# daac-tools/daachorse

Measured on AMD Instinct MI355X. Metric: haystack GB/s scanned (find_overlapping_iter(..).count(), 100k-pattern bytewise automaton), higher is better.
Workload: dtype u8/u32 integer

## Files before the change

### daachorse_amd/csrc/api_internal.hpp

```cpp
#pragma once
#include <hip/hip_runtime.h>

#include <algorithm>
#include <atomic>
#include <cassert>
#include <cstdlib>
#include <chrono>
#include <cstring>
#include <map>
#include <memory>
#include <condition_variable>
#include <deque>
#include <functional>
#include <mutex>
#include <string>
#include <thread>
#include <utility>
#include <vector>

#include "charwise.hpp"
#include "device_tables.hpp"
#include "gram.hpp"
#include "gram2.hpp"
#include "gram4.hpp"
// ... 12 lines not shown
    X(rows_share_pct, 45, 1)                                                                                                                 \
    X(blocks_per_cu, 0, 0)                                                                                                     \
    X(threads, 1024, 0)                                                                                                                      \
    X(iter_window, 64ll << 20, 0)                  \
    X(max_result_bytes, 8ll << 30, 0)                                                                                                        \
    X(gram_lds_budget, 158 * 1024, 1)                                                                                                        \
    X(gram_region, 0, 0)                                          \
    X(gram_slab, 4096, 0)                                                                                                                    \
    X(gram_ppl, 0, 0)                                                                      \
    X(gram_dense, -1, 0)                                                                                      \
    X(gram_rank_in_lds, -1, 1)                                                                                \
    X(gram_version, 0, 0)                   \
    X(gram4_arith, 1, 0)                  \
    X(gram4_filter, 1, 0)                      \
    X(gram4_mph, 8, 1)                    \
    X(gram2_dpp, 1, 0)                                                  \
    X(find3, 1, 0)                                                                                         \
    X(pfx_probe, 16384, 0)                                                             \
    X(pfx, 1, 1)                                 \
    X(gram_tail, -1, 0)                         \
    X(gram2_rfull, 1, 0)                                                            \
    X(emit, 1, 0)                            \
    X(emit_rec_per_kib, 32, 0)                               \
    X(restart_bpc, 8, 0)                                                              \
    X(restart_chain, 1, 0)                      \
    X(chain_rounds, 24, 0)                                                                                                                   \
    X(overlap_micro, 1, 0)                \
    X(pool, 1, 0)                                                                 \
    X(pool_keep, 0, 0)                                                                    \
    X(left3, 1, 0)                        \
// ... 397 lines not shown
```

### daachorse_amd/csrc/api_scan.hip

```cpp
#include "api_internal.hpp"

static daac_status scan_count_impl(daac_pma *pma, int mode, int engine, const uint8_t *hay, size_t len, size_t begin, int hay_is_device,
                                   void *stream_, uint64_t *count, uint64_t *checksum, uint64_t *result_dev, bool want_checksum);

namespace {

__global__ void repack8_kernel(const uint4 *in, uint2 *out, unsigned long long n, unsigned long long base, uint32_t end_bits) {
    for (unsigned long long i = static_cast<unsigned long long>(blockIdx.x) * blockDim.x + threadIdx.x; i < n; i += static_cast<unsigned long long>(gridDim.x) * blockDim.x) {
        const uint4 t = in[i];
        const unsigned long long end = (static_cast<unsigned long long>(t.y) << 32) | t.x;
        out[i] = uint2{t.w, static_cast<uint32_t>(end - base) | (t.z << end_bits)};
    }
}
__global__ void repack16_kernel(const daac_match *in, uint4 *out, unsigned long long n) {
    for (unsigned long long i = static_cast<unsigned long long>(blockIdx.x) * blockDim.x + threadIdx.x; i < n; i += static_cast<unsigned long long>(gridDim.x) * blockDim.x) {
        const daac_match m = in[i];
        out[i] = uint4{static_cast<uint32_t>(m.end), static_cast<uint32_t>(m.end >> 32), static_cast<uint32_t>(m.end - m.start), m.value};
    }
}

__global__ void shard_subtract_kernel(unsigned long long *r, const unsigned long long *h, unsigned long long from32) {
    r[0] -= h[0];
    r[1] -= h[1];
    r[2] -= h[2];
// ... 307 lines not shown
    return DAAC_OK;
}

daac_status stage_window(const uint8_t *host_hay, uint64_t copy_from, uint64_t end, hipStream_t stream, void **dbuf,
                         const uint8_t **virt_base) {
    const uint64_t n = end - copy_from;
    const uint64_t skew = copy_from & 15;
    HIP_TRY(hipMalloc(dbuf, n + skew + 32));
    if (n) HIP_TRY(hipMemcpyAsync(static_cast<uint8_t *>(*dbuf) + skew, host_hay + copy_from, n, hipMemcpyHostToDevice, stream));
    *virt_base = static_cast<const uint8_t *>(*dbuf) + skew - copy_from;
    return DAAC_OK;
}


static bool gram4_shape(const DeviceTables *t, CountPlan &cp) {
    const bool want_rfull = OPT(gram2_rfull) != 0, want_arith = OPT(gram4_arith) != 0, want_filter = OPT(gram4_filter) != 0;
    const uint32_t waves = static_cast<uint32_t>(OPT(threads)) > 512 ? 16u : 8u;
    const int64_t ppl_opt = OPT(gram_ppl);
    struct Shape { uint32_t ppl; bool rfull; } shapes[4] = {{32u, true}, {32u, false}, {16u, true}, {16u, false}};
    for (uint32_t w = waves; w >= 8u; w >>= 1)
        for (const Shape &sh : shapes)
            if ((sh.ppl == ppl_opt || (ppl_opt != 16 && ppl_opt != 32)) && (want_rfull || !sh.rfull) &&
                gram4_plan(t->gram4, sh.ppl, w, sh.rfull, want_arith, want_filter, 160u * 1024u, cp.g4)) { cp.ppl = sh.ppl; return true; }
    return false;
}

CountPlan resolve_count(const daac_pma *pma, const DeviceTables *t, int mode, int engine, bool want_checksum, uint64_t span) {
    CountPlan cp{};
    auto refuse = [&](const char *err, CountKernel kernel = CountKernel::walkers) { cp.kernel = kernel; cp.st = DAAC_ERR_UNSUPPORTED; cp.err = err; return cp; };
    const int64_t gv = OPT(gram_version);
    const bool g1_can = t->gram_ok && gv != 2;
    const bool g2_can = t->gram2_ok && (!want_checksum || t->gram2.exact_ok) && gv != 1 && !(gv == 0 && want_checksum && g1_can);
    const bool gw_can = t->gramw_ok && (!want_checksum || t->gramw.exact_ok);
    const bool applies = !pma->charwise && mode == DAAC_FIND_OVERLAPPING && pma->host.is_standard() && span < (1ull << 35);
    const bool gram = applies && (engine == DAAC_ENGINE_GRAM || (engine == DAAC_ENGINE_AUTO && (g2_can || g1_can || gw_can)));
    bool pfx = applies && t->pfx_ok && (engine == DAAC_ENGINE_PFX || (engine == DAAC_ENGINE_AUTO && !gram));
    cp.probe = pfx && engine == DAAC_ENGINE_AUTO && OPT(pfx_probe) != 0;
    if (cp.probe && t->pfx_dense.load() > 0) pfx = false;
// ... 28 lines not shown
std::pair<int, int> count_ids(const DeviceTables *t, const CountPlan &cp) {
    switch (cp.kernel) {
    case CountKernel::gram4: return {DAAC_ENGINE_GRAM, DAAC_KERNEL_GRAM_COUNT};
    case CountKernel::gram: case CountKernel::gram2: return {DAAC_ENGINE_GRAM, DAAC_KERNEL_GRAM_EXACT};
    case CountKernel::gram2w: return {DAAC_ENGINE_GRAM, DAAC_KERNEL_GRAM_WIDE};
    case CountKernel::pfx: return {DAAC_ENGINE_PFX, DAAC_KERNEL_PFX};
    default: return {cp.tier ? DAAC_ENGINE_TIERED : DAAC_ENGINE_DARRAY, micro_walker(t, cp.charwise, cp.tier) ? DAAC_KERNEL_MICRO : DAAC_KERNEL_SEGMENT};
    }
}

static std::string count_kernel_name(const CountPlan &cp) {
    static const char *const family[] = {"gram4", "gram", "gram2", "gram2w", "pfx"};
    if (cp.kernel == CountKernel::walkers) return cp.charwise ? "charwise" : cp.tier ? "tiered" : "darray";
    if (cp.kernel != CountKernel::gram4) return family[static_cast<int>(cp.kernel)];
    return "gram4 ppl=" + std::to_string(cp.ppl) + " dir=" + std::to_string(cp.g4.dir) + " waves=" + std::to_string(cp.g4.threads / 64) + " arith=" +
           std::to_string(cp.g4.arith) + " filter=" + std::to_string(cp.g4.filter) + " mph=" + std::to_string(cp.g4.mph) + " tail=" + (OPT(gram_tail) < 0 ? std::string("auto") : std::to_string(OPT(gram_tail) > 0 ? 1 : 0));
}

}
}

extern "C" {

static daac_status scan_count_impl(daac_pma *pma, int mode, int engine, const uint8_t *hay, size_t len, size_t begin, int hay_is_device,
                                   void *stream_, uint64_t *count, uint64_t *checksum, uint64_t *result_dev, bool want_checksum) {
    PmaScope scope_(pma);
    if (!pma || (len && !hay) || (!result_dev && (!count || (want_checksum && !checksum))) || begin > len) {
        set_error("bad argument");
        return DAAC_ERR_INVALID_ARGUMENT;
    }
    hipStream_t stream = static_cast<hipStream_t>(stream_);
// ... 409 lines not shown
```

### daachorse_amd/csrc/api_upload.hip

```cpp
#include "api_internal.hpp"

namespace {

bool recover_patterns(const HostPma &p, std::vector<uint8_t> &blob, std::vector<uint64_t> &offs, std::vector<uint32_t> &vals) {
    const uint32_t n = static_cast<uint32_t>(p.states_len());
    if (n == 0 || output_pos_of(p.opos_ch(kRoot)) != 0) return false;
    constexpr uint32_t kNone = 0xffffffffu;
    std::vector<uint32_t> depth(n, kNone), parent(n, kNone), order{kRoot};
    std::vector<uint8_t> label(n, 0);
    depth[kRoot] = 0;
    for (size_t qi = 0; qi < order.size(); ++qi) {
        const uint32_t s = order[qi], base = p.base(s);
        if (base == 0) continue;
        for (uint32_t c = 0; c < 256; ++c) {
            const uint32_t t = base ^ c;
            if (t >= n || t == kRoot || t == kDead || check_of(p.opos_ch(t)) != c) continue;
            if (depth[t] != kNone) return false;
            depth[t] = depth[s] + 1; parent[t] = s; label[t] = static_cast<uint8_t>(c);
            order.push_back(t);
        }
    }
    blob.clear(); offs.assign(1, 0); vals.clear();
    std::vector<uint8_t> tmp;
    for (const uint32_t s : order) {
// ... 314 lines not shown
            d.lds_exact = d.off_ring_exact + ring_bytes;
            if (d.off_m_exact + d.m_bytes > (1u << 17) || d.lds_exact > 160u * 1024u) exact_ok = false;
            d.K = g2.K; d.C = g2.C; d.s16 = g2.s16; d.unused_byte = g2.unused_byte;
            d.n_deep = static_cast<uint32_t>(g2.dhit.size());
            d.exact_ok = exact_ok;
            d.xlane_dpp = OPT(gram2_dpp) != 0;
            t->gram2_ok = d.off_m_count + d.m_bytes <= (1u << 17) && d.lds_count <= 160u * 1024u;
            if (t->gram2_ok) {
                Gram4Tables g4;
                build_gram4_tables(g2, g4);
                Gram4Dev &q = t->gram4;
                q = Gram4Dev{};
                if ((st = t->put(g4.cls, q.cls)) != DAAC_OK) return st;
                if ((st = t->put(g4.m, q.m)) != DAAC_OK) return st;
                q.m_bytes = p16(g4.m.size() * 4);
                if (g4.s16) {
                    std::vector<uint16_t> s16(g4.sdir.begin(), g4.sdir.end());
                    const uint16_t *ps;
                    if ((st = t->put(s16, ps)) != DAAC_OK) return st;
                    q.sdir = ps;
                    q.s_bytes = p16(s16.size() * 2);
                    if ((st = t->put(g4.rfull, q.rfull)) != DAAC_OK) return st;
                    q.rfull_bytes = p16(g4.rfull.size() * 2);
                } else {
                    const uint32_t *ps;
                    if ((st = t->put(g4.sdir, ps)) != DAAC_OK) return st;
                    q.sdir = ps;
                    q.s_bytes = p16(g4.sdir.size() * 4);
                }
                { const U32x2 *x; if ((st = t->put(g4.dhit_c, x)) != DAAC_OK) return st; q.dhit_c = reinterpret_cast<const uint2 *>(x); }
// ... 446 lines not shown
```

### daachorse_amd/csrc/device_tables.hpp

```cpp
#pragma once

#include <hip/hip_runtime.h>

#include <cstdint>

#include "../../include/daachorse_amd.h"
#include "gram4_mph.hpp"

namespace daac {

struct TierDev {
    const void *rows;
    const uint32_t *bcmap;
    const uint32_t *bfail;
    const uint2 *ssum;
    const uint8_t *cls;
    const uint4 *grec;
    const uint32_t *sopos;
    const uint32_t *outputs;
    const uint32_t *ohash;
    uint32_t C, NA, NB, N;
    uint32_t off_bcmap, off_bfail, off_ssum, off_cls, lds_bytes;
    uint32_t row32, root_flag;
};
// ... 146 lines not shown
    uint32_t v3c_bytes, v3c_dir, v3c_val;
};
hipError_t launch_gram2_scan(const Gram2Dev &dev, const GramArgs &a, bool exact, uint32_t blocks, uint32_t threads, hipStream_t stream);

struct Gram3Lds {
    uint32_t off_s;
    uint32_t off_wave;
    uint32_t wave_stride;
    uint32_t lds_bytes, threads, rfull;
};

constexpr uint32_t kGram4EndsBitDev = 30;
struct Gram4Dev {
    const uint8_t *cls;
    const uint32_t *m;
    const uint16_t *rfull;
    const void *sdir;
    const uint2 *dhit_c;
    const uint4 *dhit_t;
    const uint4 *drec_c;
    const uint4 *drec_t;
    const uint32_t *bloom;
    uint32_t bloom_words;
    const uint8_t *mph_disp;
    const uint2 *dhit_h;
    G4Mph mph;
    uint32_t mph_bytes;
    uint32_t m_bytes, rfull_bytes, s_bytes;
    uint32_t K, C, s16, arith, lo, unused_byte, n_deep;
};
struct Gram4Lds {
    uint32_t off_wave;
    uint32_t wave_stride;
    uint32_t off_cls;
    uint32_t off_s;
    uint32_t off_m;
    uint32_t s_bytes;
    uint32_t lds_bytes, threads;
    uint32_t arith;
    uint32_t dir;
    uint32_t filter;
    uint32_t off_b;
    uint32_t s_bytes_f;
    uint32_t mph;
};
uint32_t gram4_filter_room(uint32_t m_bytes, uint32_t sdir_bytes, bool arith, uint32_t lds_limit);
bool gram4_plan(const Gram4Dev &dev, uint32_t ppl, uint32_t waves, bool rfull, bool want_arith, bool want_filter, uint32_t lds_limit, Gram4Lds &L);
hipError_t launch_gram4_scan(const Gram4Dev &dev, const GramArgs &a, const Gram4Lds &L, uint32_t blocks, hipStream_t stream);

constexpr uint32_t kEmit3Tile = 1024;
constexpr uint32_t kEmit3Chunk = 1024;
constexpr uint32_t kEmit3MaxExtrasAtPosition = 15;
constexpr uint32_t kEmit3MaxExtras = 64;
constexpr uint32_t kEmit3Stage = 960;
constexpr uint32_t kEmit3ExpandWave = (kEmit3Stage + 64) * 8 + 2048 + 256 + 1024 + kEmit3MaxExtras * 16 + 16;
constexpr uint32_t kEmit3ExpandWave16 = (kEmit3Stage + 64) * 2 + 1040 + 2048 + 256 + 1024 + kEmit3MaxExtras * 16 + 16;
struct Emit3Args {
    const uint8_t *hay_al;
    uint32_t lead;
    uint32_t vlen;
    uint32_t emit_from;
    uint8_t *ann;
// ... 125 lines not shown
```

### daachorse_amd/csrc/gram4.cpp

```cpp
#include "gram4.hpp"

#include <algorithm>

namespace daac {

void build_gram4_tables(const Gram2Tables &g2, Gram4Tables &out) {
    out = Gram4Tables{};
    if (!g2.available) return;
    const uint32_t K = g2.K, C = g2.C, OTH = C - 1;
    auto perm = [&](uint32_t c) -> uint32_t { return c == 0 ? OTH : c - 1; };
    out.K = K;
    out.C = C;
    out.unused_byte = g2.unused_byte;
    out.cls.resize(256);
    for (uint32_t b = 0; b < 256; ++b) out.cls[b] = static_cast<uint8_t>(perm(g2.cls[b]));
    {
        uint32_t lo = 256;
        for (uint32_t b = 0; b < 256; ++b) if (out.cls[b] == 0) lo = b;
        bool ok = lo < 256;
        for (uint32_t b = 0; b < 256 && ok; ++b) {
            const uint32_t u = b - lo;
            ok = out.cls[b] == (u < OTH ? u : OTH);
        }
        out.arith = ok;
// ... 190 lines not shown
            if (d == 256) ok = false;
            else disp[b] = static_cast<uint8_t>(d);
        }
        if (!ok) continue;
        t.mph = p;
        t.mph_seed = seed;
        t.mph_slots = slots;
        t.mph_disp = disp;
        t.dhit_h.assign(slots, U32x2{0u, 0u});
        for (size_t i = 0; i < n; ++i) t.dhit_h[g4m_slot(h[i], f[i], disp[g4m_bucket(h[i], p)], p)] = t.dhit_c[i];
        return true;
    }
    return false;
}

}
```

### daachorse_amd/csrc/gram4.hpp

```cpp
#pragma once

#include <cstdint>
#include <vector>

#include "gram2.hpp"
#include "gram4_filter.hpp"
#include "gram4_mph.hpp"

namespace daac {

struct Gram4Tables {
    bool available = false;
    uint32_t K = 0, C = 0;
    bool arith = false;
    uint32_t lo = 0;
    uint8_t unused_byte = 0;
    bool s16 = false;
    std::vector<uint8_t> cls;
    std::vector<uint32_t> m;
    std::vector<uint16_t> rfull;
    std::vector<uint32_t> sdir;
    std::vector<U32x2> dhit_c;
    std::vector<U32x4> dhit_t, drec_c, drec_t;
    std::vector<uint32_t> bloom;
    uint32_t filter_keys = 0;
    std::vector<uint8_t> mph_disp;
    std::vector<U32x2> dhit_h;
    uint32_t mph_slots = 0, mph_seed = 0;
    G4Mph mph{};
};

constexpr uint32_t kGram4EndsBit = 30;
constexpr uint32_t kGram4ChildBits = 0x3fffffffu;

void build_gram4_tables(const Gram2Tables &g2, Gram4Tables &out);
bool build_gram4_filter(Gram4Tables &t, uint32_t max_bytes);
constexpr uint32_t kGram4MphSeeds = 8;
bool build_gram4_mph(Gram4Tables &t, uint32_t max_disp_bytes, uint32_t max_seeds = kGram4MphSeeds);

}
```

### daachorse_amd/csrc/gram4_kernels.hip

```cpp
#include <hip/hip_runtime.h>

#include <algorithm>
#include <cstdint>
#include <utility>

#include "device_tables.hpp"
#include "gram4_filter.hpp"

namespace daac {

namespace {

typedef uint32_t g4_u32x4_t __attribute__((ext_vector_type(4)));
constexpr uint32_t kList4 = 256;
constexpr uint32_t kProbePercent4 = 3;
typedef __attribute__((address_space(3))) const uint32_t lds4_cu32;
typedef __attribute__((address_space(3))) uint32_t lds4_u32;
typedef __attribute__((address_space(3))) const uint16_t lds4_cu16;
typedef __attribute__((address_space(3))) uint16_t lds4_u16;
typedef __attribute__((address_space(3))) const uint8_t lds4_cu8;
typedef __attribute__((address_space(3))) g4_u32x4_t lds4_u32x4;

__device__ __forceinline__ uint32_t pin4(uint32_t x) {
    asm("" : "+v"(x));
    return x;
}
__device__ __forceinline__ uint32_t mad24(uint32_t a, uint32_t b, uint32_t c) {
    uint32_t d;
    asm("v_mad_u32_u24 %0, %1, %2, %3" : "=v"(d) : "v"(a), "s"(b), "v"(c));
    return d;
}
__device__ __forceinline__ uint32_t wave_shr1_4(uint32_t v, uint32_t lane0) {
    uint32_t d = lane0;
    asm volatile("s_nop 1\nv_mov_b32_dpp %0, %1 wave_shr:1 row_mask:0xf bank_mask:0xf" : "+v"(d) : "v"(v));
    return d;
}
__device__ __forceinline__ uint32_t g4_wave_scan(uint32_t v) {
    v += static_cast<uint32_t>(__builtin_amdgcn_update_dpp(0, static_cast<int>(v), 0x111, 0xf, 0xf, false));
    v += static_cast<uint32_t>(__builtin_amdgcn_update_dpp(0, static_cast<int>(v), 0x112, 0xf, 0xf, false));
    v += static_cast<uint32_t>(__builtin_amdgcn_update_dpp(0, static_cast<int>(v), 0x114, 0xf, 0xf, false));
    v += static_cast<uint32_t>(__builtin_amdgcn_update_dpp(0, static_cast<int>(v), 0x118, 0xf, 0xf, false));
    v += static_cast<uint32_t>(__builtin_amdgcn_update_dpp(0, static_cast<int>(v), 0x142, 0xa, 0xf, false));
    v += static_cast<uint32_t>(__builtin_amdgcn_update_dpp(0, static_cast<int>(v), 0x143, 0xc, 0xf, false));
    return v;
}
template <typename F, int... I>
__device__ __forceinline__ void g4_turns(F &&f, std::integer_sequence<int, I...>) {
    (void)(... && f(std::integral_constant<int, I>{}));
}
__device__ __forceinline__ unsigned long long g4_wave_sum(unsigned long long v) {
#pragma unroll
    for (int off = 32; off > 0; off >>= 1) v += __shfl_down(v, off, 64);
    return v;
}
__device__ __forceinline__ void g4_copy(void *dst, const void *src, uint32_t bytes) {
    const uint4 *s = reinterpret_cast<const uint4 *>(src);
    uint4 *d = reinterpret_cast<uint4 *>(dst);
    for (uint32_t i = threadIdx.x; i < bytes / 16; i += blockDim.x) d[i] = s[i];
}
__device__ __forceinline__ void g4_reduce(unsigned long long cnt, unsigned long long *scratch, unsigned long long *result) {
    const unsigned long long c = g4_wave_sum(cnt);
    __syncthreads();
    const int wave = threadIdx.x >> 6, lane = threadIdx.x & 63;
    if (lane == 0) scratch[wave] = c;
    __syncthreads();
    if (threadIdx.x == 0) {
        unsigned long long r0 = 0;
        for (int w = 0; w < static_cast<int>((blockDim.x + 63) >> 6); ++w) r0 += scratch[w];
        if (r0) atomicAdd(result, r0);
    }
}

}

template <int K, int Q, bool ARITH, int DIR, bool TAIL, bool FILT, bool MPH = false>
__device__ __forceinline__ void gram4_body(const Gram4Dev &g, const GramArgs &a, const Gram4Lds &L, char *smem) {
    static_assert(!(FILT && TAIL), "the filter runs in front of the plain records");
    static_assert(!(FILT && DIR == 0), "the filter's Bloom array lies where the per-word directory would");
    static_assert(!MPH || FILT, "the perfect hash serves the survivors of the filter");
    constexpr int P = 16 * Q;
    constexpr int GS = 8;
    constexpr uint32_t SB = 64u * P;
    constexpr uint32_t SLOT = SB + 32u;
    const uint32_t offM = L.off_m, offS = L.off_s, offC = L.off_cls;
    const uint32_t lo = g.lo, OTH = g.C - 1u, C = g.C;
    auto cls_of = [&](uint32_t byte) -> uint32_t {
        if (ARITH) {
            const uint32_t u = byte - lo;
            return u < OTH ? u : OTH;
        }
        return *reinterpret_cast<lds4_cu8 *>(static_cast<uintptr_t>(offC + byte));
    };
    auto lds_u32 = [&](uint32_t addr) -> uint32_t { return *reinterpret_cast<lds4_cu32 *>(static_cast<uintptr_t>(addr)); };
    auto below = [&](uint32_t k) -> uint32_t { return (1u << k) - 1u; };

    const uint32_t lane = threadIdx.x & 63;
    const uint32_t lane_off = pin4(lane * (16u * Q));
    const uint32_t wave_in_wg = __builtin_amdgcn_readfirstlane(threadIdx.x >> 6);
    const uint32_t C4 = C * 4u, CC4 = C * C * 4u;
    const uint32_t ub4 = g.unused_byte * 0x01010101u;
    const uint8_t *__restrict__ hay = a.hay_al;
    const uint64_t nwaves = static_cast<uint64_t>(gridDim.x) * (blockDim.x >> 6);
    const uint32_t tb = L.off_wave + wave_in_wg * L.wave_stride;
    const uint32_t listb = wave_in_wg * (kList4 * 2u);
    const uint64_t slab_index = (static_cast<uint64_t>(blockIdx.x) * (blockDim.x >> 6) + wave_in_wg) * a.wq_slab;
    uint4 *__restrict__ slab4 = reinterpret_cast<uint4 *>(a.wq) + slab_index;
    uint32_t wq_n = 0, slab_hi = 0;
    uint64_t epoch_base = 0;
    const uint32_t drain_early = wave_in_wg * 64u;

    unsigned long long tot_cnt = 0;
    uint32_t cnt32 = 0;

    auto load_chunk = [&](uint64_t v) -> uint4 {
// ... 195 lines not shown
        if (ARITH) {
            idx = mad24((x_lo >> 8) & 0xffu, C, ((x_lo >> 16) & 0xffu) - lo_idx);
            if (K == 3) idx = mad24(x_lo & 0xffu, C * C, idx);
            d = (x_lo >> 24) - lo;
        } else {
            const uint32_t c1 = cls_of((x_lo >> 8) & 0xffu), c2 = cls_of((x_lo >> 16) & 0xffu);
            d = cls_of(x_lo >> 24);
            idx = __umul24(c1, C) + c2;
            if (K == 3) idx = __umul24(cls_of(x_lo & 0xffu), C * C) + idx;
        }
        const uint32_t am = (idx << 2) + offM;
        const uint32_t own = lds_u32(am);
        uint32_t rank;
        if (DIR == 0) {
            const uint32_t base = *reinterpret_cast<lds4_cu16 *>(static_cast<uintptr_t>((idx << 1) + offS));
            rank = base + __popc(own & below(d));
        } else {
            const uint32_t grp = am & ~15u;
            const uint32_t qx = lds_u32(grp), qy = lds_u32(grp + 4u), qz = lds_u32(grp + 8u);
            const uint32_t gi = pin4(idx >> 2);
            const uint32_t base = DIR == 1 ? *reinterpret_cast<lds4_cu16 *>(static_cast<uintptr_t>((gi << 1) + offS))
                                           : *reinterpret_cast<lds4_cu32 *>(static_cast<uintptr_t>((gi << 2) + offS));
            const uint32_t mx = static_cast<uint32_t>(__builtin_amdgcn_sbfe(static_cast<int>(0xEEEEEEEEu), idx, 1u));
            const uint32_t my = static_cast<uint32_t>(__builtin_amdgcn_sbfe(static_cast<int>(0xCCCCCCCCu), idx, 1u));
            const uint32_t mz = static_cast<uint32_t>(__builtin_amdgcn_sbfe(static_cast<int>(0x88888888u), idx, 1u));
            uint32_t under = __popc(own & below(d));
            under += __popc(qx & mx & 0x3fffffffu);
            under += __popc(qy & my & 0x3fffffffu);
            under += __popc(qz & mz & 0x3fffffffu);
            rank = base + under;
        }
        if (TAIL) {
            pend = g.dhit_t[rank];
        } else {
            const uint2 h = g.dhit_c[rank];
            pend = uint4{h.x, h.y, 0u, 0u};
        }
    };
    const G4Mph mph = g.mph;
    auto hash_and_ask = [&](uint32_t x_lo) {
        const uint32_t x = K == 3 ? x_lo : x_lo >> 8;
        const uint32_t h = g4f_h(x);
        const uint32_t d = *reinterpret_cast<lds4_cu8 *>(static_cast<uintptr_t>(offS + g4m_bucket(h, mph)));
        const uint2 r = g.dhit_h[g4m_slot(h, g4m_f(x, mph), d, mph)];
// ... 49 lines not shown
            pend_t0 = 0;
            pend_t1 = 0;
        }
        pend_valid = true;
    };

    uint64_t region = static_cast<uint64_t>(blockIdx.x) * (blockDim.x >> 6) + wave_in_wg;
    while (region < a.nregions) {
      slab_hi = static_cast<uint32_t>((region * a.region_bytes) >> 31);
      epoch_base = static_cast<uint64_t>(slab_hi) << 31;
      for (; region < a.nregions && static_cast<uint32_t>((region * a.region_bytes) >> 31) == slab_hi; region += nwaves) {
        const uint64_t rbase = region * a.region_bytes;
        const uint64_t rend = rbase + a.region_bytes < a.vlen ? rbase + a.region_bytes : a.vlen;
        uint32_t carry = 0, tail4 = 0;
#pragma unroll
        for (int i = 0; i < K; ++i) carry |= (rbase >= static_cast<uint64_t>(K - i) ? cls_of(raw_at(rbase - (K - i))) : OTH) << (8 * i);
#pragma unroll
        for (int i = 0; i < 4; ++i) tail4 |= (rbase >= static_cast<uint64_t>(4 - i) ? raw_at(rbase - (4 - i)) : static_cast<uint32_t>(g.unused_byte)) << (8 * i);
        tail4 = __builtin_amdgcn_readfirstlane(tail4);
        carry = __builtin_amdgcn_readfirstlane(carry);
        uint32_t mcarry;
        {
            uint32_t x = (((carry >> (8 * (K - 1))) & 0xffu) << 2) + offM;
            x += __umul24((carry >> (8 * (K - 2))) & 0xffu, C4);
            if (K == 3) x += __umul24(carry & 0xffu, CC4);
            mcarry = __builtin_amdgcn_readfirstlane(lds_u32(x));
        }

        const uint32_t rlen = static_cast<uint32_t>(rend - rbase);
        const uint32_t fast_lo = rbase < 16u ? SB : 0u;
        const uint32_t fast_hi = rlen & ~(SB - 1u);
        auto fetch = [&](uint32_t off, uint4 (&out)[Q]) {
            if (off >= fast_lo && off < fast_hi) {
                const uint8_t *__restrict__ base = hay + rbase + off;
                uint32_t voff = lane_off;
                asm volatile("" : "+v"(voff));
#pragma unroll
                for (int q = 0; q < Q; ++q) {
                    const g4_u32x4_t t = __builtin_nontemporal_load(reinterpret_cast<const g4_u32x4_t *>(base + voff + 16u * q));
                    out[q] = uint4{t.x, t.y, t.z, t.w};
                }
                return;
// ... 34 lines not shown
#pragma unroll
            for (int q = 0; q < Q; ++q)
                *reinterpret_cast<lds4_u32x4 *>(static_cast<uintptr_t>(my_text + 16u * q)) = g4_u32x4_t{cur[q].x, cur[q].y, cur[q].z, cur[q].w};
            if (lane == 0) {
                *reinterpret_cast<lds4_u32 *>(static_cast<uintptr_t>(slot + 12u)) = tail4;
                *reinterpret_cast<lds4_u32x4 *>(static_cast<uintptr_t>(slot + 16u + SB)) = g4_u32x4_t{pf0[0].x, pf0[0].y, pf0[0].z, pf0[0].w};
            }
            tail4 = __builtin_amdgcn_readlane(cur[Q - 1].w, 63);

            uint32_t kx[K + P];
#pragma unroll
            for (int q = 0; q < Q; ++q) {
                const uint32_t w[4] = {cur[q].x, cur[q].y, cur[q].z, cur[q].w};
#pragma unroll
                for (int b = 0; b < 16; ++b) {
                    kx[K + 16 * q + b] = pin4(cls_of((w[b >> 2] >> (8 * (b & 3))) & 0xffu));
                    __builtin_assume(kx[K + 16 * q + b] < 32u);
                }
            }
            uint32_t pk = 0;
#pragma unroll
            for (int i = 0; i < K; ++i) pk |= kx[P + i] << (8 * i);
            const uint32_t left = wave_shr1_4(pk, carry);
            carry = __builtin_amdgcn_readlane(pk, 63);
#pragma unroll
            for (int i = 0; i < K; ++i) { kx[i] = (left >> (8 * i)) & 0xffu; __builtin_assume(kx[i] < 32u); }

            uint32_t H = 0, ccnt = 0, roll = 0, mprev = 0;
#pragma unroll
            for (int grp = 0; grp < P / GS; ++grp) {
                uint32_t mw[GS];
#pragma unroll
                for (int jj = 0; jj < GS; ++jj) {
                    const int j = grp * GS + jj;
                    uint32_t x = pin4((kx[K + j] << 2) + offM);
                    x = mad24(kx[K + j - 1], C4, x);
                    if (K == 3) x = mad24(kx[K + j - 2], CC4, x);
                    mw[jj] = lds_u32(x);
                }
#pragma unroll
                for (int jj = 0; jj < GS; ++jj) {
                    const int j = grp * GS + jj;
                    roll = __builtin_amdgcn_alignbit(roll, mw[jj], 30);
                    if (j > 0) H = __builtin_amdgcn_alignbit((jj == 0 ? mprev : mw[jj - 1]) >> kx[K + j], H, 1);
                    if ((j & 15) == 15) {
                        ccnt += __popc(roll & 0x55555555u) + 2u * __popc(roll & 0xaaaaaaaau);
                        roll = 0;
                    }
                }
                mprev = mw[GS - 1];
            }
            {
                const uint32_t mleft = wave_shr1_4(mprev, mcarry);
                mcarry = __builtin_amdgcn_readlane(mprev, 63);
                H |= __builtin_amdgcn_ubfe(mleft, kx[K], 1) << (32 - P);
            }
            cnt32 += ccnt;

            const uint32_t text_adj = my_text - (32u - P) - tb;
            for (;;) {
                if (__ballot(H != 0u) == 0) break;
                const uint32_t n = __popc(H);
                const uint32_t incl = g4_wave_scan(n);
                const uint32_t tot = __builtin_amdgcn_readlane(incl, 63);
                const uint32_t first = q_tail + incl - n;
                const uint32_t room = first < kList4 ? kList4 - first : 0u;
                const uint32_t lim = n < room ? n : room;
                const uint32_t at = pin4(listb + (first << 1));
                g4_turns([&](auto tc) -> bool {
                    constexpr uint32_t t = decltype(tc)::value;
// ... 20 lines not shown
        }
        tot_cnt += cnt32;
        cnt32 = 0;
      }
      if (st_n + q_tail - q_head != 0) process_batch(st_n + q_tail - q_head);
      if (FILT && sb_n != 0) { survivors_ask(sb_n); sb_n = 0; }
      consume_pending();
      finish_second();
      drain();
      tot_cnt += cnt32;
      cnt32 = 0;
    }
    g4_reduce(tot_cnt, reinterpret_cast<unsigned long long *>(smem), a.result);
}

template <int K, int Q, bool ARITH, int DIR, int TPB, bool FILT, bool MPH = false>
__global__ __launch_bounds__(TPB) void gram4_kernel(const Gram4Dev g, const GramArgs a, const Gram4Lds L) {
    extern __shared__ __attribute__((aligned(16))) char smem[];
    constexpr int DIRC = DIR == 0 ? 1 : DIR;
    if (!ARITH) g4_copy(smem + L.off_cls, g.cls, 256);
    g4_copy(smem + L.off_m, g.m, g.m_bytes);
    uint32_t *votes = reinterpret_cast<uint32_t *>(smem + L.off_wave);
    if (threadIdx.x == 0) *votes = 0;
    __syncthreads();
    if (__builtin_amdgcn_groupstaticsize() != 0) __builtin_trap();
    bool tail = a.sel_want == 1u;
    if (a.sel_want == 2u) {
        const uint64_t span = a.vlen > a.lead + 16 ? a.vlen - a.lead - 8 : 0;
        bool go = false;
        if (span != 0) {
            unsigned long long h = (static_cast<unsigned long long>(threadIdx.x) + 1) * 0x9E3779B97F4A7C15ull;
            h ^= h >> 29;
            const uint64_t p = a.lead + 3 + (h % (span - 3));
            const uint8_t *t = a.hay_al + p;
            const uint32_t OTH = g.C - 1u;
            auto cl = [&](uint32_t b) -> uint32_t {
                if (ARITH) { const uint32_t u = b - g.lo; return u < OTH ? u : OTH; }
                return reinterpret_cast<const uint8_t *>(smem + L.off_cls)[b];
            };
            const uint32_t *m = reinterpret_cast<const uint32_t *>(smem + L.off_m);
            const uint32_t c0 = cl(t[-3]), c1 = cl(t[-2]), c2 = cl(t[-1]), d = cl(t[0]), k1 = cl(t[1]);
            const uint32_t ctx = K == 3 ? (c0 * g.C + c1) * g.C + c2 : c1 * g.C + c2;
            const uint32_t w = m[ctx];
            if ((w >> d) & 1u & (d < OTH ? 1u : 0u)) {
                uint32_t rank = __popc(w & ((1u << d) - 1u));
                for (uint32_t j = ctx & ~3u; j < ctx; ++j) rank += __popc(m[j] & 0x3fffffffu);
                rank += g.s16 ? reinterpret_cast<const uint16_t *>(g.sdir)[ctx >> 2] : reinterpret_cast<const uint32_t *>(g.sdir)[ctx >> 2];
                const uint2 r = g.dhit_c[rank];
                go = ((r.x >> k1) & 1u) != 0;
            }
        }
        const unsigned long long bm = __ballot(go);
        if ((threadIdx.x & 63) == 0 && bm != 0) atomicAdd(votes, static_cast<uint32_t>(__popcll(bm)));
        __syncthreads();
        tail = *votes * 100u > static_cast<uint32_t>(TPB) * kProbePercent4;
        __syncthreads();
    }
    if (FILT && !tail) {
        g4_copy(smem + L.off_s, MPH ? static_cast<const void *>(g.mph_disp) : g.sdir, L.s_bytes_f);
        g4_copy(smem + L.off_b, g.bloom, g.bloom_words * 4u);
    } else {
        g4_copy(smem + L.off_s, DIR == 0 ? static_cast<const void *>(g.rfull) : g.sdir, L.s_bytes);
    }
    __syncthreads();
    if (tail) gram4_body<K, Q, ARITH, DIR, true, false>(g, a, L, smem);
    else if constexpr (FILT) gram4_body<K, Q, ARITH, DIRC, false, true, MPH>(g, a, L, smem);
    else gram4_body<K, Q, ARITH, DIR, false, false>(g, a, L, smem);
}

template <int K, int Q, bool ARITH, int DIR, int TPB, bool FILT, bool MPH = false>
static hipError_t launch4_inst(const Gram4Dev &dev, const GramArgs &a, const Gram4Lds &L, uint32_t blocks, hipStream_t stream) {
    const hipError_t e = hipFuncSetAttribute(reinterpret_cast<const void *>(gram4_kernel<K, Q, ARITH, DIR, TPB, FILT, MPH>),
                                             hipFuncAttributeMaxDynamicSharedMemorySize, static_cast<int>(L.lds_bytes));
    if (e != hipSuccess) return e;
    hipLaunchKernelGGL((gram4_kernel<K, Q, ARITH, DIR, TPB, FILT, MPH>), dim3(blocks), dim3(TPB), L.lds_bytes, stream, dev, a, L);
    return hipGetLastError();
}
template <int K, int Q, int TPB, bool ARITH>
static hipError_t launch4_d(const Gram4Dev &dev, const GramArgs &a, const Gram4Lds &L, uint32_t blocks, hipStream_t stream) {
    if (L.filter && L.mph) {
        if (L.dir == 0) return launch4_inst<K, Q, ARITH, 0, TPB, true, true>(dev, a, L, blocks, stream);
        if (L.dir == 1) return launch4_inst<K, Q, ARITH, 1, TPB, true, true>(dev, a, L, blocks, stream);
        return launch4_inst<K, Q, ARITH, 2, TPB, true, true>(dev, a, L, blocks, stream);
    }
    if (L.filter) {
        if (L.dir == 0) return launch4_inst<K, Q, ARITH, 0, TPB, true>(dev, a, L, blocks, stream);
        if (L.dir == 1) return launch4_inst<K, Q, ARITH, 1, TPB, true>(dev, a, L, blocks, stream);
        return launch4_inst<K, Q, ARITH, 2, TPB, true>(dev, a, L, blocks, stream);
    }
    if (L.dir == 0) return launch4_inst<K, Q, ARITH, 0, TPB, false>(dev, a, L, blocks, stream);
    if (L.dir == 1) return launch4_inst<K, Q, ARITH, 1, TPB, false>(dev, a, L, blocks, stream);
    return launch4_inst<K, Q, ARITH, 2, TPB, false>(dev, a, L, blocks, stream);
}
template <int K, int Q, int TPB>
static hipError_t launch4_k(const Gram4Dev &dev, const GramArgs &a, const Gram4Lds &L, uint32_t blocks, hipStream_t stream) {
    return L.arith ? launch4_d<K, Q, TPB, true>(dev, a, L, blocks, stream) : launch4_d<K, Q, TPB, false>(dev, a, L, blocks, stream);
}

bool gram4_plan(const Gram4Dev &dev, uint32_t ppl, uint32_t waves, bool rfull, bool want_arith, bool want_filter, uint32_t lds_limit, Gram4Lds &L) {
    L = Gram4Lds{};
    if (rfull && dev.rfull == nullptr) return false;
    const uint32_t slot = 64u * ppl + 32u;
    L.wave_stride = slot;
    L.off_wave = waves * kList4 * 2u;
    L.threads = waves * 64u;
    L.arith = (want_arith && dev.arith) ? 1u : 0u;
    const uint32_t per_wg = L.off_wave + waves * L.wave_stride;
    L.off_cls = per_wg;
    L.off_s = per_wg + (L.arith ? 0u : 256u);
    L.dir = rfull ? 0u : (dev.s16 ? 1u : 2u);
    L.s_bytes = rfull ? dev.rfull_bytes : dev.s_bytes;
    uint32_t region = L.s_bytes;
    if (want_filter && dev.bloom != nullptr) {
        const uint32_t front = dev.mph_disp != nullptr ? dev.mph_bytes : dev.s_bytes;
        const uint32_t with = front + dev.bloom_words * 4u;
        if (L.off_s + std::max(region, with) + dev.m_bytes <= lds_limit) {
            L.filter = 1u;
            L.mph = dev.mph_disp != nullptr ? 1u : 0u;
            L.s_bytes_f = front;
            L.off_b = L.off_s + front;
            region = std::max(region, with);
// ... 23 lines not shown
```

Baseline: 1701.

## Add bit-reversed gram4 mask layout so match counts accumulate by integer addition

Builds an alternative gram4 table in which each context word holds its count in the low five bits and its child bits reversed into the high bits. Class codes are inverted and addressing uses negative signed 24-bit multiply-adds. This lets the scan kernel add up eight mask words per group and read the hit count from the low bits, replacing the per-word alignbit/popcount roll accumulation. It costs an extra device table, a new set of kernel template instantiations, and changed rank and bit-test arithmetic in the filter and directory paths, limited to C<=27.

```diff
diff --git a/daachorse_amd/csrc/api_internal.hpp b/daachorse_amd/csrc/api_internal.hpp
--- a/daachorse_amd/csrc/api_internal.hpp
+++ b/daachorse_amd/csrc/api_internal.hpp
@@ -50,6 +50,7 @@
     X(gram4_arith, 1, 0)                  \
     X(gram4_filter, 1, 0)                      \
     X(gram4_mph, 8, 1)                    \
+    X(gram4_add, 1, 0)                    \
     X(gram2_dpp, 1, 0)                                                  \
     X(find3, 1, 0)                                                                                         \
     X(pfx_probe, 16384, 0)                                                             \
diff --git a/daachorse_amd/csrc/api_scan.hip b/daachorse_amd/csrc/api_scan.hip
--- a/daachorse_amd/csrc/api_scan.hip
+++ b/daachorse_amd/csrc/api_scan.hip
@@ -345,14 +345,14 @@
 
 
 static bool gram4_shape(const DeviceTables *t, CountPlan &cp) {
-    const bool want_rfull = OPT(gram2_rfull) != 0, want_arith = OPT(gram4_arith) != 0, want_filter = OPT(gram4_filter) != 0;
+    const bool want_rfull = OPT(gram2_rfull) != 0, want_arith = OPT(gram4_arith) != 0, want_filter = OPT(gram4_filter) != 0, want_add = OPT(gram4_add) != 0;
     const uint32_t waves = static_cast<uint32_t>(OPT(threads)) > 512 ? 16u : 8u;
     const int64_t ppl_opt = OPT(gram_ppl);
     struct Shape { uint32_t ppl; bool rfull; } shapes[4] = {{32u, true}, {32u, false}, {16u, true}, {16u, false}};
     for (uint32_t w = waves; w >= 8u; w >>= 1)
         for (const Shape &sh : shapes)
             if ((sh.ppl == ppl_opt || (ppl_opt != 16 && ppl_opt != 32)) && (want_rfull || !sh.rfull) &&
-                gram4_plan(t->gram4, sh.ppl, w, sh.rfull, want_arith, want_filter, 160u * 1024u, cp.g4)) { cp.ppl = sh.ppl; return true; }
+                gram4_plan(t->gram4, sh.ppl, w, sh.rfull, want_arith, want_filter, want_add, 160u * 1024u, cp.g4)) { cp.ppl = sh.ppl; return true; }
     return false;
 }
 
@@ -411,7 +411,7 @@
     if (cp.kernel == CountKernel::walkers) return cp.charwise ? "charwise" : cp.tier ? "tiered" : "darray";
     if (cp.kernel != CountKernel::gram4) return family[static_cast<int>(cp.kernel)];
     return "gram4 ppl=" + std::to_string(cp.ppl) + " dir=" + std::to_string(cp.g4.dir) + " waves=" + std::to_string(cp.g4.threads / 64) + " arith=" +
-           std::to_string(cp.g4.arith) + " filter=" + std::to_string(cp.g4.filter) + " mph=" + std::to_string(cp.g4.mph) + " tail=" + (OPT(gram_tail) < 0 ? std::string("auto") : std::to_string(OPT(gram_tail) > 0 ? 1 : 0));
+           std::to_string(cp.g4.arith) + " filter=" + std::to_string(cp.g4.filter) + " mph=" + std::to_string(cp.g4.mph) + " add=" + std::to_string(cp.g4.add) + " tail=" + (OPT(gram_tail) < 0 ? std::string("auto") : std::to_string(OPT(gram_tail) > 0 ? 1 : 0));
 }
 
 }
diff --git a/daachorse_amd/csrc/api_upload.hip b/daachorse_amd/csrc/api_upload.hip
--- a/daachorse_amd/csrc/api_upload.hip
+++ b/daachorse_amd/csrc/api_upload.hip
@@ -352,6 +352,10 @@
                 if ((st = t->put(g4.cls, q.cls)) != DAAC_OK) return st;
                 if ((st = t->put(g4.m, q.m)) != DAAC_OK) return st;
                 q.m_bytes = p16(g4.m.size() * 4);
+                {
+                    std::vector<uint32_t> m_add;
+                    if (build_gram4_add(g4, m_add) && (st = t->put(m_add, q.m_add)) != DAAC_OK) return st;
+                }
                 if (g4.s16) {
                     std::vector<uint16_t> s16(g4.sdir.begin(), g4.sdir.end());
                     const uint16_t *ps;
diff --git a/daachorse_amd/csrc/device_tables.hpp b/daachorse_amd/csrc/device_tables.hpp
--- a/daachorse_amd/csrc/device_tables.hpp
+++ b/daachorse_amd/csrc/device_tables.hpp
@@ -184,6 +184,7 @@
 struct Gram4Dev {
     const uint8_t *cls;
     const uint32_t *m;
+    const uint32_t *m_add;
     const uint16_t *rfull;
     const void *sdir;
     const uint2 *dhit_c;
@@ -213,9 +214,10 @@
     uint32_t off_b;
     uint32_t s_bytes_f;
     uint32_t mph;
+    uint32_t add;
 };
 uint32_t gram4_filter_room(uint32_t m_bytes, uint32_t sdir_bytes, bool arith, uint32_t lds_limit);
-bool gram4_plan(const Gram4Dev &dev, uint32_t ppl, uint32_t waves, bool rfull, bool want_arith, bool want_filter, uint32_t lds_limit, Gram4Lds &L);
+bool gram4_plan(const Gram4Dev &dev, uint32_t ppl, uint32_t waves, bool rfull, bool want_arith, bool want_filter, bool want_add, uint32_t lds_limit, Gram4Lds &L);
 hipError_t launch_gram4_scan(const Gram4Dev &dev, const GramArgs &a, const Gram4Lds &L, uint32_t blocks, hipStream_t stream);
 
 constexpr uint32_t kEmit3Tile = 1024;
diff --git a/daachorse_amd/csrc/gram4.cpp b/daachorse_amd/csrc/gram4.cpp
--- a/daachorse_amd/csrc/gram4.cpp
+++ b/daachorse_amd/csrc/gram4.cpp
@@ -228,4 +228,12 @@
     return false;
 }
 
-}
+bool build_gram4_add(const Gram4Tables &t, std::vector<uint32_t> &m_add) {
+    m_add.clear();
+    if (!t.available || t.C > kGram4AddMaxC) return false;
+    m_add.resize(t.m.size());
+    for (size_t i = 0; i < t.m.size(); ++i) m_add[i] = gram4_add_word(t.m[i]);
+    return true;
+}
+
+}
diff --git a/daachorse_amd/csrc/gram4.hpp b/daachorse_amd/csrc/gram4.hpp
--- a/daachorse_amd/csrc/gram4.hpp
+++ b/daachorse_amd/csrc/gram4.hpp
@@ -38,4 +38,17 @@
 constexpr uint32_t kGram4MphSeeds = 8;
 bool build_gram4_mph(Gram4Tables &t, uint32_t max_disp_bytes, uint32_t max_seeds = kGram4MphSeeds);
 
+constexpr uint32_t kGram4AddMaxC = 27;
+constexpr uint32_t kGram4AddCountMask = 31u;
+inline uint32_t gram4_brev32(uint32_t x) {
+    x = ((x >> 1) & 0x55555555u) | ((x & 0x55555555u) << 1);
+    x = ((x >> 2) & 0x33333333u) | ((x & 0x33333333u) << 2);
+    x = ((x >> 4) & 0x0f0f0f0fu) | ((x & 0x0f0f0f0fu) << 4);
+    x = ((x >> 8) & 0x00ff00ffu) | ((x & 0x00ff00ffu) << 8);
+    return (x >> 16) | (x << 16);
 }
+inline uint32_t gram4_add_word(uint32_t m) { return (m >> 30) | gram4_brev32(m & kGram4ChildBits); }
+inline uint32_t gram4_add_word_back(uint32_t a) { return (a << 30) | gram4_brev32(a & ~kGram4AddCountMask); }
+bool build_gram4_add(const Gram4Tables &t, std::vector<uint32_t> &m_add);
+
+}
diff --git a/daachorse_amd/csrc/gram4_kernels.hip b/daachorse_amd/csrc/gram4_kernels.hip
--- a/daachorse_amd/csrc/gram4_kernels.hip
+++ b/daachorse_amd/csrc/gram4_kernels.hip
@@ -6,6 +6,10 @@
 
 #include "device_tables.hpp"
 #include "gram4_filter.hpp"
+
+#ifndef DAAC_G4_ADD3
+#define DAAC_G4_ADD3 0
+#endif
 
 namespace daac {
 
@@ -30,6 +34,21 @@
     asm("v_mad_u32_u24 %0, %1, %2, %3" : "=v"(d) : "v"(a), "s"(b), "v"(c));
     return d;
 }
+__device__ __forceinline__ uint32_t madi24(uint32_t a, uint32_t b, uint32_t c) {
+    uint32_t d;
+    asm("v_mad_i32_i24 %0, %1, %2, %3" : "=v"(d) : "v"(a), "s"(b), "v"(c));
+    return d;
+}
+__device__ __forceinline__ uint32_t g4_add2(uint32_t a, uint32_t b) {
+    uint32_t d;
+    asm("v_add_u32 %0, %1, %2" : "=v"(d) : "v"(a), "v"(b));
+    return d;
+}
+__device__ __forceinline__ uint32_t g4_add3(uint32_t a, uint32_t b, uint32_t c) {
+    uint32_t d;
+    asm("v_add3_u32 %0, %1, %2, %3" : "=v"(d) : "v"(a), "v"(b), "v"(c));
+    return d;
+}
 __device__ __forceinline__ uint32_t wave_shr1_4(uint32_t v, uint32_t lane0) {
     uint32_t d = lane0;
     asm volatile("s_nop 1\nv_mov_b32_dpp %0, %1 wave_shr:1 row_mask:0xf bank_mask:0xf" : "+v"(d) : "v"(v));
@@ -57,6 +76,11 @@
     const uint4 *s = reinterpret_cast<const uint4 *>(src);
     uint4 *d = reinterpret_cast<uint4 *>(dst);
     for (uint32_t i = threadIdx.x; i < bytes / 16; i += blockDim.x) d[i] = s[i];
+}
+__device__ __forceinline__ void g4_copy_not(void *dst, const void *src, uint32_t bytes) {
+    const uint4 *s = reinterpret_cast<const uint4 *>(src);
+    uint4 *d = reinterpret_cast<uint4 *>(dst);
+    for (uint32_t i = threadIdx.x; i < bytes / 16; i += blockDim.x) { const uint4 v = s[i]; d[i] = uint4{~v.x, ~v.y, ~v.z, ~v.w}; }
 }
 __device__ __forceinline__ void g4_reduce(unsigned long long cnt, unsigned long long *scratch, unsigned long long *result) {
     const unsigned long long c = g4_wave_sum(cnt);
@@ -73,7 +97,7 @@
 
 }
 
-template <int K, int Q, bool ARITH, int DIR, bool TAIL, bool FILT, bool MPH = false>
+template <int K, int Q, bool ARITH, int DIR, bool TAIL, bool FILT, bool MPH = false, bool ADD = false>
 __device__ __forceinline__ void gram4_body(const Gram4Dev &g, const GramArgs &a, const Gram4Lds &L, char *smem) {
     static_assert(!(FILT && TAIL), "the filter runs in front of the plain records");
     static_assert(!(FILT && DIR == 0), "the filter's Bloom array lies where the per-word directory would");
@@ -89,15 +113,46 @@
             const uint32_t u = byte - lo;
             return u < OTH ? u : OTH;
         }
+        const uint32_t c = *reinterpret_cast<lds4_cu8 *>(static_cast<uintptr_t>(offC + byte));
+        return ADD ? c ^ 0xffu : c;
+    };
+    const uint32_t lo1 = lo - 1u, nOTH = ~OTH;
+    auto cword_of = [&](uint32_t byte) -> uint32_t {
+        if (!ADD) return cls_of(byte);
+        if (ARITH) {
+            const uint32_t u = lo1 - byte;
+            return u > nOTH ? u : nOTH;
+        }
         return *reinterpret_cast<lds4_cu8 *>(static_cast<uintptr_t>(offC + byte));
+    };
+    const uint32_t wbase = ARITH ? ~0u : 255u;
+    auto cword_unpack = [&](uint32_t packed, int i) -> uint32_t {
+        if (ADD && ARITH) return static_cast<uint32_t>(static_cast<int32_t>(packed << (24 - 8 * i)) >> 24);
+        return (packed >> (8 * i)) & 0xffu;
     };
     auto lds_u32 = [&](uint32_t addr) -> uint32_t { return *reinterpret_cast<lds4_cu32 *>(static_cast<uintptr_t>(addr)); };
     auto below = [&](uint32_t k) -> uint32_t { return (1u << k) - 1u; };
+    auto m_below = [&](uint32_t d) -> uint32_t { return ADD ? ~(0xffffffffu >> d) : below(d); };
+    constexpr uint32_t kChild = ADD ? ~31u : 0x3fffffffu;
 
     const uint32_t lane = threadIdx.x & 63;
     const uint32_t lane_off = pin4(lane * (16u * Q));
     const uint32_t wave_in_wg = __builtin_amdgcn_readfirstlane(threadIdx.x >> 6);
     const uint32_t C4 = C * 4u, CC4 = C * C * 4u;
+    const uint32_t nC4 = 0u - C4, nCC4 = 0u - CC4, n4 = 0u - 4u;
+    const uint32_t offMr = offM + wbase * (4u + C4 + (K == 3 ? CC4 : 0u));
+    auto m_addr = [&](uint32_t w0, uint32_t w1, uint32_t w2) -> uint32_t {
+        if (ADD) {
+            uint32_t x = madi24(w0, n4, offMr);
+            x = madi24(w1, nC4, x);
+            if (K == 3) x = madi24(w2, nCC4, x);
+            return x;
+        }
+        uint32_t x = pin4((w0 << 2) + offM);
+        x = mad24(w1, C4, x);
+        if (K == 3) x = mad24(w2, CC4, x);
+        return x;
+    };
     const uint32_t ub4 = g.unused_byte * 0x01010101u;
     const uint8_t *__restrict__ hay = a.hay_al;
     const uint64_t nwaves = static_cast<uint64_t>(gridDim.x) * (blockDim.x >> 6);
@@ -323,7 +378,7 @@
         uint32_t rank;
         if (DIR == 0) {
             const uint32_t base = *reinterpret_cast<lds4_cu16 *>(static_cast<uintptr_t>((idx << 1) + offS));
-            rank = base + __popc(own & below(d));
+            rank = base + __popc(own & m_below(d));
         } else {
             const uint32_t grp = am & ~15u;
             const uint32_t qx = lds_u32(grp), qy = lds_u32(grp + 4u), qz = lds_u32(grp + 8u);
@@ -333,10 +388,10 @@
             const uint32_t mx = static_cast<uint32_t>(__builtin_amdgcn_sbfe(static_cast<int>(0xEEEEEEEEu), idx, 1u));
             const uint32_t my = static_cast<uint32_t>(__builtin_amdgcn_sbfe(static_cast<int>(0xCCCCCCCCu), idx, 1u));
             const uint32_t mz = static_cast<uint32_t>(__builtin_amdgcn_sbfe(static_cast<int>(0x88888888u), idx, 1u));
-            uint32_t under = __popc(own & below(d));
-            under += __popc(qx & mx & 0x3fffffffu);
-            under += __popc(qy & my & 0x3fffffffu);
-            under += __popc(qz & mz & 0x3fffffffu);
+            uint32_t under = __popc(own & m_below(d));
+            under += __popc(qx & mx & kChild);
+            under += __popc(qy & my & kChild);
+            under += __popc(qz & mz & kChild);
             rank = base + under;
         }
         if (TAIL) {
@@ -416,18 +471,13 @@
         const uint64_t rend = rbase + a.region_bytes < a.vlen ? rbase + a.region_bytes : a.vlen;
         uint32_t carry = 0, tail4 = 0;
 #pragma unroll
-        for (int i = 0; i < K; ++i) carry |= (rbase >= static_cast<uint64_t>(K - i) ? cls_of(raw_at(rbase - (K - i))) : OTH) << (8 * i);
+        for (int i = 0; i < K; ++i) carry |= ((rbase >= static_cast<uint64_t>(K - i) ? cword_of(raw_at(rbase - (K - i))) : (ADD ? wbase - OTH : OTH)) & 0xffu) << (8 * i);
 #pragma unroll
         for (int i = 0; i < 4; ++i) tail4 |= (rbase >= static_cast<uint64_t>(4 - i) ? raw_at(rbase - (4 - i)) : static_cast<uint32_t>(g.unused_byte)) << (8 * i);
         tail4 = __builtin_amdgcn_readfirstlane(tail4);
         carry = __builtin_amdgcn_readfirstlane(carry);
         uint32_t mcarry;
-        {
-            uint32_t x = (((carry >> (8 * (K - 1))) & 0xffu) << 2) + offM;
-            x += __umul24((carry >> (8 * (K - 2))) & 0xffu, C4);
-            if (K == 3) x += __umul24(carry & 0xffu, CC4);
-            mcarry = __builtin_amdgcn_readfirstlane(lds_u32(x));
-        }
+        mcarry = __builtin_amdgcn_readfirstlane(lds_u32(m_addr(cword_unpack(carry, K - 1), cword_unpack(carry, K - 2), K == 3 ? cword_unpack(carry, 0) : 0u)));
 
         const uint32_t rlen = static_cast<uint32_t>(rend - rbase);
         const uint32_t fast_lo = rbase < 16u ? SB : 0u;
@@ -492,46 +542,57 @@
                 const uint32_t w[4] = {cur[q].x, cur[q].y, cur[q].z, cur[q].w};
 #pragma unroll
                 for (int b = 0; b < 16; ++b) {
-                    kx[K + 16 * q + b] = pin4(cls_of((w[b >> 2] >> (8 * (b & 3))) & 0xffu));
-                    __builtin_assume(kx[K + 16 * q + b] < 32u);
+                    kx[K + 16 * q + b] = pin4(cword_of((w[b >> 2] >> (8 * (b & 3))) & 0xffu));
+                    if (!ADD) __builtin_assume(kx[K + 16 * q + b] < 32u);
                 }
             }
             uint32_t pk = 0;
 #pragma unroll
-            for (int i = 0; i < K; ++i) pk |= kx[P + i] << (8 * i);
+            for (int i = 0; i < K; ++i) pk |= (ADD ? kx[P + i] & 0xffu : kx[P + i]) << (8 * i);
             const uint32_t left = wave_shr1_4(pk, carry);
             carry = __builtin_amdgcn_readlane(pk, 63);
 #pragma unroll
-            for (int i = 0; i < K; ++i) { kx[i] = (left >> (8 * i)) & 0xffu; __builtin_assume(kx[i] < 32u); }
-
-            uint32_t H = 0, ccnt = 0, roll = 0, mprev = 0;
+            for (int i = 0; i < K; ++i) { kx[i] = cword_unpack(left, i); if (!ADD) __builtin_assume(kx[i] < 32u); }
+
+            uint32_t H = 0, ccnt = 0, roll = 0, acc = 0, mprev = 0;
 #pragma unroll
             for (int grp = 0; grp < P / GS; ++grp) {
                 uint32_t mw[GS];
 #pragma unroll
                 for (int jj = 0; jj < GS; ++jj) {
                     const int j = grp * GS + jj;
-                    uint32_t x = pin4((kx[K + j] << 2) + offM);
-                    x = mad24(kx[K + j - 1], C4, x);
-                    if (K == 3) x = mad24(kx[K + j - 2], CC4, x);
-                    mw[jj] = lds_u32(x);
+                    mw[jj] = lds_u32(m_addr(kx[K + j], kx[K + j - 1], K == 3 ? kx[K + j - 2] : 0u));
                 }
 #pragma unroll
                 for (int jj = 0; jj < GS; ++jj) {
                     const int j = grp * GS + jj;
-                    roll = __builtin_amdgcn_alignbit(roll, mw[jj], 30);
-                    if (j > 0) H = __builtin_amdgcn_alignbit((jj == 0 ? mprev : mw[jj - 1]) >> kx[K + j], H, 1);
-                    if ((j & 15) == 15) {
+                    if (!ADD) roll = __builtin_amdgcn_alignbit(roll, mw[jj], 30);
+                    if (j > 0) H = __builtin_amdgcn_alignbit((jj == 0 ? mprev : mw[jj - 1]) >> (ADD ? kx[K + j] & 31u : kx[K + j]), H, 1);
+                    if (!ADD && (j & 15) == 15) {
                         ccnt += __popc(roll & 0x55555555u) + 2u * __popc(roll & 0xaaaaaaaau);
                         roll = 0;
                     }
                 }
+                if (ADD) {
+#if DAAC_G4_ADD3
+                    static_assert(GS == 8, "three v_add3_u32 and one v_add_u32 a group");
+                    acc = g4_add3(mw[0], mw[1], mw[2]);
+                    acc = g4_add3(acc, mw[3], mw[4]);
+                    acc = g4_add3(acc, mw[5], mw[6]);
+                    acc = g4_add2(acc, mw[7]);
+#else
+                    acc = g4_add2(mw[0], mw[1]);
+#pragma unroll
+                    for (int jj = 2; jj < GS; ++jj) acc = g4_add2(acc, mw[jj]);
+#endif
+                    ccnt += acc & 31u;
+                }
                 mprev = mw[GS - 1];
             }
             {
                 const uint32_t mleft = wave_shr1_4(mprev, mcarry);
                 mcarry = __builtin_amdgcn_readlane(mprev, 63);
-                H |= __builtin_amdgcn_ubfe(mleft, kx[K], 1) << (32 - P);
+                H |= __builtin_amdgcn_ubfe(mleft, ADD ? kx[K] & 31u : kx[K], 1) << (32 - P);
             }
             cnt32 += ccnt;
 
@@ -582,12 +643,12 @@
     g4_reduce(tot_cnt, reinterpret_cast<unsigned long long *>(smem), a.result);
 }
 
-template <int K, int Q, bool ARITH, int DIR, int TPB, bool FILT, bool MPH = false>
+template <int K, int Q, bool ARITH, int DIR, int TPB, bool FILT, bool MPH = false, bool ADD = false>
 __global__ __launch_bounds__(TPB) void gram4_kernel(const Gram4Dev g, const GramArgs a, const Gram4Lds L) {
     extern __shared__ __attribute__((aligned(16))) char smem[];
     constexpr int DIRC = DIR == 0 ? 1 : DIR;
-    if (!ARITH) g4_copy(smem + L.off_cls, g.cls, 256);
-    g4_copy(smem + L.off_m, g.m, g.m_bytes);
+    if (!ARITH) { if (ADD) g4_copy_not(smem + L.off_cls, g.cls, 256); else g4_copy(smem + L.off_cls, g.cls, 256); }
+    g4_copy(smem + L.off_m, ADD ? g.m_add : g.m, g.m_bytes);
     uint32_t *votes = reinterpret_cast<uint32_t *>(smem + L.off_wave);
     if (threadIdx.x == 0) *votes = 0;
     __syncthreads();
@@ -604,15 +665,16 @@
             const uint32_t OTH = g.C - 1u;
             auto cl = [&](uint32_t b) -> uint32_t {
                 if (ARITH) { const uint32_t u = b - g.lo; return u < OTH ? u : OTH; }
-                return reinterpret_cast<const uint8_t *>(smem + L.off_cls)[b];
+                const uint32_t c = reinterpret_cast<const uint8_t *>(smem + L.off_cls)[b];
+                return ADD ? c ^ 0xffu : c;
             };
             const uint32_t *m = reinterpret_cast<const uint32_t *>(smem + L.off_m);
             const uint32_t c0 = cl(t[-3]), c1 = cl(t[-2]), c2 = cl(t[-1]), d = cl(t[0]), k1 = cl(t[1]);
             const uint32_t ctx = K == 3 ? (c0 * g.C + c1) * g.C + c2 : c1 * g.C + c2;
             const uint32_t w = m[ctx];
-            if ((w >> d) & 1u & (d < OTH ? 1u : 0u)) {
-                uint32_t rank = __popc(w & ((1u << d) - 1u));
-                for (uint32_t j = ctx & ~3u; j < ctx; ++j) rank += __popc(m[j] & 0x3fffffffu);
+            if ((w >> (ADD ? 31u - d : d)) & 1u & (d < OTH ? 1u : 0u)) {
+                uint32_t rank = __popc(w & (ADD ? ~(0xffffffffu >> d) : (1u << d) - 1u));
+                for (uint32_t j = ctx & ~3u; j < ctx; ++j) rank += __popc(m[j] & (ADD ? ~31u : 0x3fffffffu));
                 rank += g.s16 ? reinterpret_cast<const uint16_t *>(g.sdir)[ctx >> 2] : reinterpret_cast<const uint32_t *>(g.sdir)[ctx >> 2];
                 const uint2 r = g.dhit_c[rank];
                 go = ((r.x >> k1) & 1u) != 0;
@@ -631,18 +693,26 @@
         g4_copy(smem + L.off_s, DIR == 0 ? static_cast<const void *>(g.rfull) : g.sdir, L.s_bytes);
     }
     __syncthreads();
-    if (tail) gram4_body<K, Q, ARITH, DIR, true, false>(g, a, L, smem);
-    else if constexpr (FILT) gram4_body<K, Q, ARITH, DIRC, false, true, MPH>(g, a, L, smem);
-    else gram4_body<K, Q, ARITH, DIR, false, false>(g, a, L, smem);
-}
-
+    if (tail) gram4_body<K, Q, ARITH, DIR, true, false, false, ADD>(g, a, L, smem);
+    else if constexpr (FILT) gram4_body<K, Q, ARITH, DIRC, false, true, MPH, ADD>(g, a, L, smem);
+    else gram4_body<K, Q, ARITH, DIR, false, false, false, ADD>(g, a, L, smem);
+}
+
+template <int K, int Q, bool ARITH, int DIR, int TPB, bool FILT, bool MPH, bool ADD>
+static hipError_t launch4_layout(const Gram4Dev &dev, const GramArgs &a, const Gram4Lds &L, uint32_t blocks, hipStream_t stream) {
+    const hipError_t e = hipFuncSetAttribute(reinterpret_cast<const void *>(gram4_kernel<K, Q, ARITH, DIR, TPB, FILT, MPH, ADD>),
+                                             hipFuncAttributeMaxDynamicSharedMemorySize, static_cast<int>(L.lds_bytes));
+    if (e != hipSuccess) return e;
+    hipLaunchKernelGGL((gram4_kernel<K, Q, ARITH, DIR, TPB, FILT, MPH, ADD>), dim3(blocks), dim3(TPB), L.lds_bytes, stream, dev, a, L);
+    return hipGetLastError();
+}
 template <int K, int Q, bool ARITH, int DIR, int TPB, bool FILT, bool MPH = false>
 static hipError_t launch4_inst(const Gram4Dev &dev, const GramArgs &a, const Gram4Lds &L, uint32_t blocks, hipStream_t stream) {
-    const hipError_t e = hipFuncSetAttribute(reinterpret_cast<const void *>(gram4_kernel<K, Q, ARITH, DIR, TPB, FILT, MPH>),
-                                             hipFuncAttributeMaxDynamicSharedMemorySize, static_cast<int>(L.lds_bytes));
-    if (e != hipSuccess) return e;
-    hipLaunchKernelGGL((gram4_kernel<K, Q, ARITH, DIR, TPB, FILT, MPH>), dim3(blocks), dim3(TPB), L.lds_bytes, stream, dev, a, L);
-    return hipGetLastError();
+    if (L.add) {
+        if (dev.m_add == nullptr) return hipErrorInvalidValue;
+        return launch4_layout<K, Q, ARITH, DIR, TPB, FILT, MPH, true>(dev, a, L, blocks, stream);
+    }
+    return launch4_layout<K, Q, ARITH, DIR, TPB, FILT, MPH, false>(dev, a, L, blocks, stream);
 }
 template <int K, int Q, int TPB, bool ARITH>
 static hipError_t launch4_d(const Gram4Dev &dev, const GramArgs &a, const Gram4Lds &L, uint32_t blocks, hipStream_t stream) {
@@ -665,7 +735,7 @@
     return L.arith ? launch4_d<K, Q, TPB, true>(dev, a, L, blocks, stream) : launch4_d<K, Q, TPB, false>(dev, a, L, blocks, stream);
 }
 
-bool gram4_plan(const Gram4Dev &dev, uint32_t ppl, uint32_t waves, bool rfull, bool want_arith, bool want_filter, uint32_t lds_limit, Gram4Lds &L) {
+bool gram4_plan(const Gram4Dev &dev, uint32_t ppl, uint32_t waves, bool rfull, bool want_arith, bool want_filter, bool want_add, uint32_t lds_limit, Gram4Lds &L) {
     L = Gram4Lds{};
     if (rfull && dev.rfull == nullptr) return false;
     const uint32_t slot = 64u * ppl + 32u;
@@ -673,6 +743,7 @@
     L.off_wave = waves * kList4 * 2u;
     L.threads = waves * 64u;
     L.arith = (want_arith && dev.arith) ? 1u : 0u;
+    L.add = (want_add && dev.m_add != nullptr) ? 1u : 0u;
     const uint32_t per_wg = L.off_wave + waves * L.wave_stride;
     L.off_cls = per_wg;
     L.off_s = per_wg + (L.arith ? 0u : 256u);
```

Result: no change. 1696 (-0.3%).
